# discere-os/zlib.wasm

Hardware: AMD Instinct MI355X
Metric: compress MB/s @ level 6 + CRC32 GB/s, batched 1 MB buffers, 1/2/4/8 GPU (higher is better)
Workload: dtype u8; 1 GPU; C4 per-GPU shard: 32768 x 1048576 B buffers per GPU, deflate level 6, zlib wrapper, inputs+outputs in HBM; level=6, buffer_bytes=1048576, buffers_per_gpu=32768, inflight_mb=4096, parallelism=1 GPU(s), one rank each, buffers sharded by index, no data-path collective, world_size_seen=1

## Files before the change

zlib.wasm_amd/csrc/zgpu_deflate.hip:

```cpp
#include "zgpu_internal.h"
#include <cstdlib>
#include <cstdio>

namespace zgpu {

__constant__ CodeTables c_ct;

constexpr uint32_t kParseFallback = 0xffffffffu;

__device__ inline uint32_t hash3(uint32_t b0, uint32_t b1, uint32_t b2) {
    return ((b0 & 31u) << 10) ^ (b1 << 5) ^ b2;
}
__device__ inline uint32_t hashp(uint32_t b0, uint32_t b1, uint32_t b2, const WinP &w) {
    return ((b0 << (2 * w.shift)) ^ (b1 << w.shift) ^ b2) & w.mask;
}
__device__ inline WinP job_win(const DeflateJob &job) { return win_params(job.wbits, job.hbits); }

__device__ inline uint32_t lds32u(const uint8_t *base, int off) {
    const uint32_t *w = reinterpret_cast<const uint32_t *>(base + (off & ~3));
    return __builtin_amdgcn_alignbyte(w[1], w[0], (uint32_t)(off & 3));
}


template <int kThreads, int kMaxChunksPerThread>
// ... 117 lines not shown
    __syncthreads();
#pragma unroll
    for (int k = 0; k < 4; k++) {
        const int idx = tid * 4 + k;
        wcnt[idx & (kLWaves - 1)][idx >> 4] = (uint16_t)run;
        run += v[k];
    }
    __syncthreads();
#pragma unroll
    for (int j = 0; j < kLPer; j++) {
        const int e = wave * (64 * kLPer) + j * 64 + lane;
        if (e < m) dst[wcnt[wave][(key[j] >> shift) & 0xffu] + rank[j]] = key[j];
    }
    __syncthreads();
}

template <int kC, int kH, bool kSegs, bool kGH>
__device__ __attribute__((always_inline)) inline void links_body(const DeflateJob &job) {
    static_assert(kC <= kLC && (kC & (kC - 1)) == 0 && kC >= 32, "chunk");
    static_assert(!kGH || (!kSegs && kH == 32768), "global head: the default layout, whole buffers");
    __shared__ uint16_t head[kGH ? 1 : kH];
    __shared__ uint32_t ka[kC];
    __shared__ __attribute__((aligned(16))) uint16_t lk[kC];
    uint8_t *const stage = reinterpret_cast<uint8_t *>(lk);
    __shared__ uint16_t wcnt[kLWaves][256];
    __shared__ int wsum[kLWaves];
    const int tid = threadIdx.x;
    const uint32_t bi = kSegs ? job.seg[2 * blockIdx.x] : blockIdx.x;
    const uint32_t g = job.first + bi;
    const int64_t n = (int64_t)job.src_len[g];
    const uint8_t *in = job.src + job.src_off[g];
    uint16_t *out = job.link + job.ws_off[bi];
    const WinP wp = job_win(job);
    const int64_t s0 = kSegs ? (int64_t)job.seg[2 * blockIdx.x + 1] : 0;
    const int64_t s1 = kSegs && s0 + (int64_t)job.seg_len < n ? s0 + (int64_t)job.seg_len : n;
    const int64_t t0 = kSegs && s0 > 32768 ? (s0 - 32768) / kC * kC : 0;

    uint32_t *const ghead = kGH ? reinterpret_cast<uint32_t *>(job.key + job.ws_off[bi]) : nullptr;
    if constexpr (kGH)
        for (int i = tid; i < kH; i += kLThreads) ghead[i] = (uint32_t)-32768;
    else
        for (int i = tid; i < kH; i += kLThreads) head[i] = (uint16_t)((t0 - 32768) & 0xffff);
    const int64_t lk_n = !kSegs && !kGH && job.lk_head ? (int64_t)job.lk_n : 0;
    for (int64_t c0 = t0; c0 < s1; c0 += kC) {
        __syncthreads();
        if (c0 + kC <= lk_n) continue;
        if (kGH) {
        } else if (c0 <= lk_n && job.lk_head) {
            const int hn = (int)wp.mask + 1;
            for (int i = tid; i < kH; i += kLThreads) {
                const int64_t q = i < hn ? (int64_t)job.lk_head[i] : 0;
                head[i] = (uint16_t)(q != 0 && c0 - q < 32768 ? q & 0xffff : (c0 - 32768) & 0xffff);
            }
            __syncthreads();
        } else if ((c0 & 32767) == 0 && c0 > 0) {
            const uint32_t now = (uint32_t)c0;
            for (int i = tid; i < kH; i += kLThreads) {
                const uint32_t age = (now - head[i]) & 0xffffu;
                if (age == 0 || age >= 32768u) head[i] = (uint16_t)((now - 32768u) & 0xffffu);
            }
        }
        stage_bytes<kLThreads, (kC + 16) / 16 / kLThreads + 1>(stage, in, c0, kC + 16, n, tid);
        __syncthreads();
        const int cnt = (int)((n - c0) < kC ? (n - c0) : kC);
        const int m = (int)((n - 2 - c0) < kC ? ((n - 2 - c0) > 0 ? n - 2 - c0 : 0) : kC);
        const int e0 = lk_n > c0 ? (int)(lk_n - c0) : 0;
        const int ms = m > e0 ? m - e0 : 0;
        for (int e = e0 + tid; e < m; e += kLThreads) {
            uint32_t h = hashp(stage[e], stage[e + 1], stage[e + 2], wp);
            if (job.sk.n) {
                const uint32_t p = (uint32_t)c0 + (uint32_t)e;
                for (uint32_t k = 0; k < job.sk.n; k++)
                    if (p >= job.sk.a[k] && p < job.sk.b[k]) h = kSkipHash;
            }
            ka[e - e0] = h << 13 | (uint32_t)e;
        }
        links_radix_pass(ka, ka, ms, 13, wcnt, wsum, tid);
        links_radix_pass(ka, ka, ms, 21, wcnt, wsum, tid);
        for (int i = tid; i < ms; i += kLThreads) {
            const uint32_t key = ka[i];
            const uint32_t h = key >> 13, e = key & (kLC - 1);
            const uint32_t p = (uint32_t)c0 + e;
            uint32_t d;
            if (h == kSkipHash) d = 0;
            else if (i > 0 && (ka[i - 1] >> 13) == h) d = e - (ka[i - 1] & (kLC - 1));
            else if (kGH) d = p - ghead[h];
            else d = (p - head[h]) & 0xffffu;
            lk[e] = (uint16_t)((d != 0 && d <= 32767u && d != p) ? d : 0u);
        }
        __syncthreads();
        for (int i = tid; i < ms; i += kLThreads) {
            const uint32_t key = ka[i];
            if ((key >> 13) != kSkipHash && (i == ms - 1 || (ka[i + 1] >> 13) != (key >> 13))) {
                if (kGH) ghead[key >> 13] = (uint32_t)c0 + (key & (kLC - 1));
                else head[key >> 13] = (uint16_t)(((uint32_t)c0 + (key & (kLC - 1))) & 0xffffu);
            }
        }
        if (kSegs) {
            const int w0 = s0 > c0 ? (int)(s0 - c0) : 0, w1 = (int)(s1 - c0 < cnt ? s1 - c0 : cnt);
            for (int e = tid + w0; e < w1; e += kLThreads) out[c0 + e] = e < m ? lk[e] : (uint16_t)0;
        } else {
            for (int e = tid + e0; e < cnt; e += kLThreads) out[c0 + e] = e < m ? lk[e] : (uint16_t)0;
        }
    }
}

template <int kC, int kH, bool kSegs = false>
__global__ __launch_bounds__(kLThreads) void k_links(DeflateJob job) {
    links_body<kC, kH, kSegs, false>(job);
}

__global__ __launch_bounds__(kLThreads, 8) void k_links_gh(DeflateJob job) {
    links_body<kLC, 32768, false, true>(job);
}

constexpr int kLS1C = 2048;
constexpr int64_t kLS1Max = 16384;
__global__ __launch_bounds__(kLThreads) void k_links_seg1(DeflateJob job) {
    __shared__ uint32_t head[32768];
    __shared__ uint32_t ka[kLS1C];
    __shared__ __attribute__((aligned(16))) uint16_t lk[kLS1C + 16];
    uint8_t *const stage = reinterpret_cast<uint8_t *>(lk);
    __shared__ uint16_t wcnt[kLWaves][256];
    __shared__ int wsum[kLWaves];
    const int tid = threadIdx.x;
    const uint32_t bi = job.seg[2 * blockIdx.x];
    const uint32_t g = job.first + bi;
    const int64_t n = (int64_t)job.src_len[g];
    const uint8_t *in = job.src + job.src_off[g];
    uint16_t *out = job.link + job.ws_off[bi];
    const WinP wp = job_win(job);
    const int64_t s0 = (int64_t)job.seg[2 * blockIdx.x + 1];
    const int64_t s1 = s0 + (int64_t)job.seg_len < n ? s0 + (int64_t)job.seg_len : n;
    auto skipped = [&](int64_t p) {
        for (uint32_t k = 0; k < job.sk.n; k++)
            if ((uint64_t)p >= job.sk.a[k] && (uint64_t)p < job.sk.b[k]) return true;
        return false;
    };
    for (int i = tid; i < 32768; i += kLThreads) head[i] = 0;
    __syncthreads();
    {
        const int64_t w0 = s0 - 32767 > 1 ? s0 - 32767 : 1, w1 = s0 < n - 2 ? s0 : n - 2;
        const int64_t q0 = w0 + 32ll * tid;
        if (q0 < w1) {
            uint32_t wb[9];
            const uintptr_t a = reinterpret_cast<uintptr_t>(in + q0);
            const uint32_t sh = (uint32_t)(a & 3u);
            const uint32_t *qw = reinterpret_cast<const uint32_t *>(a & ~(uintptr_t)3);
            const int64_t lim = n - q0;
            uint32_t d[10];
#pragma unroll
            for (int j = 0; j < 10; j++)
                d[j] = 4ll * j - (int64_t)sh < lim ? qw[j] : 0u;
#pragma unroll
            for (int j = 0; j < 9; j++) wb[j] = sh ? __builtin_amdgcn_alignbyte(d[j + 1], d[j], sh) : d[j];
#pragma unroll
            for (int j = 0; j < 32; j++) {
                const int64_t q = q0 + j;
                if (q >= w1) break;
                const uint32_t b0 = (wb[j >> 2] >> (8 * (j & 3))) & 0xffu;
                const uint32_t b1 = (wb[(j + 1) >> 2] >> (8 * ((j + 1) & 3))) & 0xffu;
                const uint32_t b2 = (wb[(j + 2) >> 2] >> (8 * ((j + 2) & 3))) & 0xffu;
                if (job.sk.n && skipped(q)) continue;
                atomicMax(&head[hashp(b0, b1, b2, wp)], (uint32_t)q + 1u);
            }
        }
    }
    for (int64_t c0 = s0; c0 < s1; c0 += kLS1C) {
        __syncthreads();
        stage_bytes<kLThreads, 1>(stage, in, c0, ((kLS1C + 16) / 16) * 16, n, tid);
        __syncthreads();
        const int cnt = (int)((s1 - c0) < kLS1C ? (s1 - c0) : kLS1C);
        const int m = (int)((n - 2 - c0) < cnt ? ((n - 2 - c0) > 0 ? n - 2 - c0 : 0) : cnt);
        for (int e = tid; e < m; e += kLThreads) {
            uint32_t h = hashp(stage[e], stage[e + 1], stage[e + 2], wp);
            if (job.sk.n && skipped(c0 + e)) h = kSkipHash;
            ka[e] = h << 11 | (uint32_t)e;
        }
        links_radix_pass(ka, ka, m, 11, wcnt, wsum, tid);
        links_radix_pass(ka, ka, m, 19, wcnt, wsum, tid);
        for (int i = tid; i < m; i += kLThreads) {
            const uint32_t key = ka[i];
            const uint32_t h = key >> 11, e = key & (kLS1C - 1);
            const int64_t p = c0 + e;
            int64_t dd;
            if (h == kSkipHash) dd = 0;
            else if (i > 0 && (ka[i - 1] >> 11) == h) dd = e - (ka[i - 1] & (kLS1C - 1));
            else dd = head[h] ? p - ((int64_t)head[h] - 1) : 0;
            lk[e] = (uint16_t)(dd > 0 && dd <= 32767 && dd != p ? dd : 0);
        }
        __syncthreads();
        for (int i = tid; i < m; i += kLThreads) {
            const uint32_t key = ka[i];
            if ((key >> 11) != kSkipHash && (i == m - 1 || (ka[i + 1] >> 11) != (key >> 11)))
                head[key >> 11] = (uint32_t)(c0 + (key & (kLS1C - 1))) + 1u;
        }
        for (int e = tid; e < cnt; e += kLThreads) out[c0 + e] = e < m ? lk[e] : (uint16_t)0;
    }
}

constexpr int kCntStage = 4096;
constexpr int kCntThreads = 1024;

__device__ __attribute__((always_inline)) inline uint32_t walk_key(uint32_t c, uint32_t chain) {
    if (c > chain) c = chain;
    if (c < 128) return c;
    const uint32_t k = 128 + ((c - 128) >> 5);
    return k < 255 ? k : 255;
}

template <bool kSegs = false>
__global__ __launch_bounds__(kCntThreads) void k_count(DeflateJob job) {
    __shared__ uint32_t cnt[16384];
    __shared__ __attribute__((aligned(16))) uint8_t s_in[kCntStage + 16];
    __shared__ __attribute__((aligned(16))) uint8_t s_out[kCntStage + 16];
    const int tid = threadIdx.x;
    const uint32_t bi = kSegs ? job.seg[2 * blockIdx.x] : blockIdx.x;
    const uint32_t g = job.first + bi;
    const int64_t n = (int64_t)job.src_len[g];
    const uint8_t *in = job.src + job.src_off[g];
    uint8_t *key = job.key + job.ws_off[bi];
    const uint32_t chain = job.cfg.chain;
    const int64_t s0 = kSegs ? (int64_t)job.seg[2 * blockIdx.x + 1] : 0;
    const int64_t s1 = kSegs && s0 + (int64_t)job.seg_len < n ? s0 + (int64_t)job.seg_len : n;
    const int64_t c0 = kSegs && s0 > kMaxDist ? (s0 - kMaxDist) / kCntStage * kCntStage : 0;
    for (int i = tid; i < 16384; i += kCntThreads) cnt[i] = 0;
    int64_t tstart = c0;
    if (kSegs && s0 > 0) {
        static_assert(kMaxDist <= 32 * kCntThreads, "one pass");
        __syncthreads();
        const int64_t w0 = s0 - kMaxDist > 1 ? s0 - kMaxDist : 1;
        const int64_t q0 = w0 + 32ll * tid;
        if (q0 < s0) {
            const uintptr_t a = reinterpret_cast<uintptr_t>(in + q0);
            const uint32_t sh = (uint32_t)(a & 3u);
            const uint32_t *qw = reinterpret_cast<const uint32_t *>(a & ~(uintptr_t)3);
            const int64_t lim = n - q0;
            uint32_t d[10], wb[9];
#pragma unroll
            for (int j = 0; j < 10; j++) d[j] = 4ll * j - (int64_t)sh < lim ? qw[j] : 0u;
#pragma unroll
            for (int j = 0; j < 9; j++) wb[j] = sh ? __builtin_amdgcn_alignbyte(d[j + 1], d[j], sh) : d[j];
#pragma unroll
            for (int j = 0; j < 32; j++) {
                const int64_t q = q0 + j;
                if (q >= s0 || q + 3 > n) break;
                const uint32_t h = hash3((wb[j >> 2] >> (8 * (j & 3))) & 0xffu,
                                         (wb[(j + 1) >> 2] >> (8 * ((j + 1) & 3))) & 0xffu,
                                         (wb[(j + 2) >> 2] >> (8 * ((j + 2) & 3))) & 0xffu);
                atomicAdd(&cnt[h >> 1], 1u << ((h & 1u) * 16));
            }
        }
        tstart = s0;
    }
    for (int64_t t0 = tstart; t0 < s1; t0 += kCntStage) {
        __syncthreads();
        stage_bytes<kCntThreads, (kCntStage + 16) / 16 / kCntThreads + 1>(s_in, in, t0, kCntStage + 16, n, tid);
        stage_bytes<kCntThreads, (kCntStage + 16) / 16 / kCntThreads + 1>(s_out, in, t0 - kMaxDist,
                                                                         kCntStage + 16, n, tid);
        __syncthreads();
        const int64_t tend = (t0 + kCntStage < n) ? t0 + kCntStage : n;
        for (int64_t p = t0 + tid; p < tend; p += kCntThreads) {
            const int j = (int)(p - t0);
            const int64_t q = p - kMaxDist;
            if (q >= 1 && q >= c0 && q + 3 <= n) {
                const uint32_t h = hash3(s_out[j], s_out[j + 1], s_out[j + 2]);
                atomicSub(&cnt[h >> 1], 1u << ((h & 1u) * 16));
            }
            uint32_t k = 0;
            if (p >= 1 && p + 3 <= n) {
                const uint32_t h = hash3(s_in[j], s_in[j + 1], s_in[j + 2]);
                const uint32_t old = atomicAdd(&cnt[h >> 1], 1u << ((h & 1u) * 16));
                k = walk_key((old >> ((h & 1u) * 16)) & 0xffffu, chain);
            }
            if (!kSegs || (p >= s0 && p < s1)) key[p] = (uint8_t)k;
        }
    }
}

constexpr int kMW = 32768, kMT = 4096, kMPad = 272;
static_assert(kMT == (int)kMatchTile, "segment starts (host) must be k_match tile boundaries");
constexpr int kME = kMW + kMT + kMPad;
constexpr int kMatchThreads = 1024;

__device__ inline uint32_t get4(const uint32_t *E, int i) {
    return (E[i] >> 16) | (E[i + 2] & 0xffff0000u);
}

__device__ inline uint32_t nil_link(uint32_t l) { return l ? l : 0xffffu; }

static_assert(kMT / 4 == kMatchThreads && kMPad % 4 == 0 && kMPad / 4 <= kMatchThreads && kMW % 4 == 0,
              "tile prefetch: 4 words per thread");
struct TilePre {
    uint32_t b[4];
    uint32_t pb[4];
    uint32_t lk[4];
    uint32_t key[4];
};

__device__ __attribute__((always_inline)) inline uint32_t ldb(const uint8_t *in, int64_t q, int64_t n) {
    return (q >= 0 && q < n) ? (uint32_t)in[q] : 0u;
}

__device__ __attribute__((always_inline)) inline void tile_prefetch(TilePre &P, int64_t ts, int64_t n,
                                                                    const uint8_t *in, const uint16_t *L,
                                                                    const uint8_t *K, int tid) {
    const int64_t q0 = ts + 4 * tid;
    uint32_t x[5];
#pragma unroll
    for (int u = 0; u < 5; u++) x[u] = ldb(in, q0 + u, n);
#pragma unroll
    for (int u = 0; u < 4; u++) P.b[u] = x[u] | x[u + 1] << 8;
    if (tid < kMPad / 4) {
        const int64_t q1 = ts + kMT + 4 * tid;
#pragma unroll
        for (int u = 0; u < 5; u++) x[u] = ldb(in, q1 + u, n);
#pragma unroll
        for (int u = 0; u < 4; u++) P.pb[u] = x[u] | x[u + 1] << 8;
    }
    if (q0 + 4 <= n) {
        const uint2 v = *reinterpret_cast<const uint2 *>(L + q0);
        P.lk[0] = v.x & 0xffffu; P.lk[1] = v.x >> 16; P.lk[2] = v.y & 0xffffu; P.lk[3] = v.y >> 16;
    } else {
#pragma unroll
        for (int u = 0; u < 4; u++) P.lk[u] = q0 + u < n ? (uint32_t)L[q0 + u] : 0u;
    }
    if (K) {
#pragma unroll
        for (int u = 0; u < 4; u++) {
            const int64_t q = ts + tid + u * kMatchThreads;
            P.key[u] = q < n ? (uint32_t)K[q] : 0u;
        }
    }
}

__device__ __attribute__((always_inline)) inline uint32_t slide_idx(uint32_t w) {
    typedef unsigned short us2 __attribute__((ext_vector_type(2)));
    const us2 v = __builtin_bit_cast(us2, w);
    const us2 d = {(unsigned short)kMT, (unsigned short)0};
    return __builtin_bit_cast(uint32_t, __builtin_elementwise_sub_sat(v, d));
}
template <bool kIdx = false>
__device__ __attribute__((always_inline)) inline void tile_store(uint32_t *E, const TilePre &P, int64_t ts,
                                                                 int tid) {
    if (ts == 0) {
        for (int i = tid; i < kMW; i += kMatchThreads) E[i] = 0;
    } else {
        uint4 *dE = reinterpret_cast<uint4 *>(E);
        for (int c = tid; c < kMW / 4; c += kMatchThreads) {
            uint4 v = dE[c + kMT / 4];
            if (kIdx) v = make_uint4(slide_idx(v.x), slide_idx(v.y), slide_idx(v.z), slide_idx(v.w));
            dE[c] = v;
        }
        __syncthreads();
    }
    const int w0 = kMW + 4 * tid;
    uint4 v;
    if (kIdx) {
        v.x = P.b[0] << 16 | (P.lk[0] ? ((uint32_t)(w0 + 0) - P.lk[0]) & 0xffffu : 0u);
        v.y = P.b[1] << 16 | (P.lk[1] ? ((uint32_t)(w0 + 1) - P.lk[1]) & 0xffffu : 0u);
        v.z = P.b[2] << 16 | (P.lk[2] ? ((uint32_t)(w0 + 2) - P.lk[2]) & 0xffffu : 0u);
        v.w = P.b[3] << 16 | (P.lk[3] ? ((uint32_t)(w0 + 3) - P.lk[3]) & 0xffffu : 0u);
    } else {
        v.x = P.b[0] << 16 | nil_link(P.lk[0]);
        v.y = P.b[1] << 16 | nil_link(P.lk[1]);
        v.z = P.b[2] << 16 | nil_link(P.lk[2]);
        v.w = P.b[3] << 16 | nil_link(P.lk[3]);
    }
    *reinterpret_cast<uint4 *>(E + w0) = v;
    if (tid < kMPad / 4)
        *reinterpret_cast<uint4 *>(E + kMW + kMT + 4 * tid) =
            make_uint4(P.pb[0] << 16, P.pb[1] << 16, P.pb[2] << 16, P.pb[3] << 16);
}

struct Scan16 { uint32_t s0, s1, s2, s3; };


constexpr int kD0 = 2;
constexpr int kDQ = 6;
constexpr int kDU = 3;
__device__ inline uint32_t ufl(uint32_t v) { return (uint32_t)__builtin_amdgcn_readfirstlane((int)v); }

__device__ __attribute__((always_inline)) inline uint32_t get4p(const uint32_t *E, int i) {
    return __builtin_amdgcn_perm(E[i + 2], E[i], 0x07060302u);
}

__device__ __attribute__((always_inline)) inline uint32_t ffbl(uint32_t x) {
    uint32_t r;
    asm("v_ffbl_b32 %0, %1" : "=v"(r) : "v"(x));
    return r;
}

__device__ __attribute__((always_inline)) inline int diff16(uint32_t x0, uint32_t x1, uint32_t x2, uint32_t x3) {
    const uint32_t b = min(min(ffbl(x0), ffbl(x1) | 32u), min(ffbl(x2) | 64u, ffbl(x3) | 96u));
    return (int)(min(b, 128u) >> 3);
}

__device__ __attribute__((always_inline)) inline int lcp16(const uint32_t *E, int m, int s, const Scan16 &S,
                                                           int maxcmp) {
    int k = diff16(get4p(E, m) ^ S.s0, get4p(E, m + 4) ^ S.s1, get4p(E, m + 8) ^ S.s2, get4p(E, m + 12) ^ S.s3);
    if (k >= 16) {
        while (k < maxcmp) {
            const int r = diff16(get4p(E, m + k) ^ get4p(E, s + k), get4p(E, m + k + 4) ^ get4p(E, s + k + 4),
                                 get4p(E, m + k + 8) ^ get4p(E, s + k + 8), get4p(E, m + k + 12) ^ get4p(E, s + k + 12));
            k += r;
            if (r < 16) break;
        }
    }
    return k < maxcmp ? k : maxcmp;
}
__device__ __attribute__((always_inline)) inline void lcp16x2(const uint32_t *E, int m1, int m0, int s,
                                                              const Scan16 &S, int maxcmp, int &l1, int &l0) {
    const uint32_t a0 = get4p(E, m1) ^ S.s0, a1 = get4p(E, m1 + 4) ^ S.s1, a2 = get4p(E, m1 + 8) ^ S.s2,
                   a3 = get4p(E, m1 + 12) ^ S.s3;
    const uint32_t b0 = get4p(E, m0) ^ S.s0, b1 = get4p(E, m0 + 4) ^ S.s1, b2 = get4p(E, m0 + 8) ^ S.s2,
                   b3 = get4p(E, m0 + 12) ^ S.s3;
    int k1 = diff16(a0, a1, a2, a3), k0 = diff16(b0, b1, b2, b3);
    auto more = [&](int m, int k) {
        while (k < maxcmp) {
            const int r = diff16(get4p(E, m + k) ^ get4p(E, s + k), get4p(E, m + k + 4) ^ get4p(E, s + k + 4),
                                 get4p(E, m + k + 8) ^ get4p(E, s + k + 8), get4p(E, m + k + 12) ^ get4p(E, s + k + 12));
            k += r;
            if (r < 16) break;
        }
        return k;
    };
    if (k1 >= 16) k1 = more(m1, k1);
    if (k0 >= 16) k0 = more(m0, k0);
    l1 = k1 < maxcmp ? k1 : maxcmp;
    l0 = k0 < maxcmp ? k0 : maxcmp;
}
__device__ inline uint32_t match_rec(int best, int s4, int bpos4) {
    return best >= kMinMatch ? (((uint32_t)best << 16) | (uint32_t)((s4 - bpos4) >> 2)) : 0u;
}


#ifdef ZGPU_MATCH_STATS
__device__ unsigned long long g_mstat[8];
#define MSTAT(i, v) atomicAdd(&g_mstat[i], (unsigned long long)(v))
#define MSTATW(i, v) do { if ((int)__lane_id() == __builtin_ctzll(__ballot(1))) atomicAdd(&g_mstat[i], (unsigned long long)(v)); } while (0)
extern "C" int zgpu_match_stats_read(unsigned long long *out, int reset) {
    if (hipMemcpyFromSymbol(out, HIP_SYMBOL(g_mstat), sizeof(g_mstat)) != hipSuccess) return -1;
    if (reset) {
        unsigned long long z[8] = {0, 0, 0, 0, 0, 0, 0, 0};
        if (hipMemcpyToSymbol(HIP_SYMBOL(g_mstat), z, sizeof(z)) != hipSuccess) return -1;
    }
    return 0;
}
#endif

struct DWQ {
    int m4, limit4, be4, occ;
    int q[kDQ];
    uint32_t em, eb, scan01, scanE;
};
__device__ __attribute__((always_inline)) inline void dwq_steps(DWQ &w, const char *Eb, uint32_t &count,
                                                                uint32_t end) {
    auto step = [&]() {
        const int m4n = (int)((w.em << 2) & 0x3fffcu);
        const uint32_t emn = *reinterpret_cast<const uint32_t *>(Eb + m4n);
        const uint32_t ebn = *reinterpret_cast<const uint32_t *>(Eb + m4n + w.be4);
        const bool pass = (w.m4 > w.limit4) & ((w.em >> 16) == w.scan01) & ((w.eb >> 16) == w.scanE);
#pragma unroll
        for (int j = kDQ - 1; j > 0; j--) w.q[j] = pass ? w.q[j - 1] : w.q[j];
        w.q[0] = pass ? w.m4 : w.q[0];
        w.occ += pass ? 1 : 0;
        w.m4 = m4n;
        w.em = emn;
        w.eb = ebn;
    };
    for (;;) {
        if (end - count >= (uint32_t)kDU) {
#pragma unroll
            for (int u = 0; u < kDU; u++) step();
            count += kDU;
        } else {
            step();
            count += 1;
        }
        const uint64_t walkers = __ballot(w.m4 > w.limit4), full = __ballot(w.occ >= kDQ - (kDU - 1));
        if (count >= end || walkers == 0 || full != 0) break;
    }
}

constexpr uint32_t kQDiff = 1u << 31;
struct MOutRQ {
    uint32_t *rf, *rq;
    int64_t p;
    mutable uint32_t q = 0;
    mutable bool hq = false;
    __device__ __attribute__((always_inline)) inline void full(uint32_t r, bool) const {
        const bool d = hq && q != r;
        if (d) rq[p] = q;
        rf[p] = d ? r | kQDiff : r;
    }
    __device__ __attribute__((always_inline)) inline void quart(uint32_t r) const {
        q = r;
        hq = true;
    }
    __device__ __attribute__((always_inline)) inline void steps(uint32_t) const {}
};
template <typename Out>
__device__ __attribute__((always_inline)) inline void dwq_walk(const uint32_t *E, int64_t p, int64_t B, int64_t n,
                                                               const LevelCfg &cfg, const Out &out,
                                                               int want_q, int64_t max_dist) {
    const int s = (int)(p - B);
    const uint32_t e0 = E[s];
    const uint32_t d0 = (e0 & 0xffffu) ? (uint32_t)s - (e0 & 0xffffu) : 0xffffu;
    if (d0 > (uint32_t)max_dist) {
        if (want_q) out.quart(0u);
        out.full(0u, true);
        return;
    }
    const int64_t labs = p > max_dist ? p - max_dist : 0;
    const int limit4 = (int)(labs - B) * 4;
    const int64_t rem = n - p;
    const int nice = rem < cfg.nice ? (int)rem : cfg.nice;
    const int maxcmp = rem < kMaxMatch ? (int)rem : kMaxMatch;
    const uint32_t chain = (uint32_t)cfg.chain;
    const uint32_t qc = want_q ? chain >> 2 : chain;
    const int s4 = s * 4;
    const Scan16 S{get4(E, s), get4(E, s + 4), get4(E, s + 8), get4(E, s + 12)};
    int best = kMinMatch - 1, bpos4 = 0;
    int m4 = (int)(e0 & 0xffffu) * 4;
    uint32_t count = 0;
    bool walking = true;
    bool need_q = want_q != 0;
#pragma unroll
    for (int k = 0; k < kD0; k++) {
        if (walking) {
            const int m = m4 >> 2;
            const uint32_t em = E[m];
            const int len = lcp16(E, m, s, S, maxcmp);
            if (len > best) { best = len; bpos4 = m4; }
            count++;
            const int m4n = (int)((em & 0xffffu) << 2);
            if (best >= nice || m4n <= limit4 || count >= chain) walking = false;
            if (need_q && count == qc && walking) {
                out.quart(match_rec(best, s4, bpos4));
                need_q = false;
            }
            m4 = m4n;
        }
    }
    if (!walking) {
        const uint32_t r = match_rec(best, s4, bpos4);
        if (need_q) out.quart(r);
        out.steps(count);
        out.full(r, best >= nice || m4 <= limit4);
        return;
    }
    const char *Eb = reinterpret_cast<const char *>(E);
#ifdef ZGPU_MATCH_STATS
    MSTATW(4, 1);
    MSTAT(6, 1);
#endif
    DWQ w;
    w.m4 = m4;
    w.limit4 = limit4;
    w.be4 = (best - 1) * 4;
    w.occ = 0;
#pragma unroll
    for (int j = 0; j < kDQ; j++) w.q[j] = 0;
    w.scan01 = e0 >> 16;
    w.scanE = E[s + best - 1] >> 16;
    w.em = *reinterpret_cast<const uint32_t *>(Eb + m4);
    w.eb = *reinterpret_cast<const uint32_t *>(Eb + m4 + w.be4);
    count = ufl(count);
    for (;;) {
        const uint32_t end = count < qc ? qc : chain;
        const int best0 = best;
        dwq_steps(w, Eb, count, end);
        walking = w.m4 > limit4 && count < chain;
#ifdef ZGPU_MATCH_STATS
        MSTATW(0, 1);
        MSTAT(2, (uint64_t)w.occ);
        MSTAT(3, 1);
#endif
        static_assert(kDQ % 2 == 0, "entries are taken in pairs");
#pragma unroll
        for (int j = kDQ - 1; j >= 1; j -= 2) {
            const bool c1 = j < w.occ, c0 = j - 1 < w.occ;
            if (__ballot(c0) != 0) {
                int l1, l0;
                lcp16x2(E, c1 ? w.q[j] >> 2 : 0, c0 ? w.q[j - 1] >> 2 : 0, s, S, maxcmp, l1, l0);
#ifdef ZGPU_MATCH_STATS
                MSTATW(1, 1);
                MSTAT(5, (c1 && l1 >= 16 ? 1 : 0) + (c0 && l0 >= 16 ? 1 : 0));
#endif
                if (c1 && l1 > best) {
                    best = l1;
                    bpos4 = w.q[j];
                    if (l1 >= nice) { walking = false; w.occ = 0; }
                }
                if (c0 && j - 1 < w.occ && l0 > best) {
                    best = l0;
                    bpos4 = w.q[j - 1];
                    if (l0 >= nice) { walking = false; w.occ = 0; }
                }
            }
        }
        w.occ = 0;
        const bool fin = !walking;
        if (need_q && (count >= qc || fin)) {
            out.quart(match_rec(best, s4, bpos4));
            need_q = false;
        }
        if (fin) break;
        if (best != best0) {
            w.be4 = (best - 1) * 4;
            w.scanE = E[s + best - 1] >> 16;
            w.eb = *reinterpret_cast<const uint32_t *>(Eb + w.m4 + w.be4);
        }
    }
    out.steps(count);
    out.full(match_rec(best, s4, bpos4), best >= nice || w.m4 <= limit4);
}


struct FlushEv {
    const uint64_t *pos;
    const uint32_t *type;
    const uint64_t *aux;
    uint32_t n, i;
    __device__ inline bool at(int64_t p) const {
        return i < n && kind() != 0 && kind() != kEvPause && kind() != kEvPrime && (int64_t)ufl64(pos[i]) == p;
    }
    __device__ inline bool prime() const { return i < n && kind() == kEvPrime; }
    __device__ inline uint32_t prime_arg() const { return (uint32_t)ufl64(aux[i]); }
    __device__ inline bool stop_at(int64_t e, int64_t lim) const { return i < n && kind() == 0 && e == lim; }
    __device__ inline bool pause_at(int64_t x) const {
        return i < n && kind() == kEvPause && (int64_t)ufl64(aux[i]) == x;
    }
    __device__ inline uint32_t kind() const { return (uint32_t)__builtin_amdgcn_readfirstlane((int)type[i]); }
    __device__ inline int64_t limit(int64_t end) const { return i < n ? (int64_t)ufl64(pos[i]) : end; }
    __device__ static inline uint64_t ufl64(uint64_t v) {
        const uint32_t lo = (uint32_t)__builtin_amdgcn_readfirstlane((int)(uint32_t)v);
        const uint32_t hi = (uint32_t)__builtin_amdgcn_readfirstlane((int)(uint32_t)(v >> 32));
        return ((uint64_t)hi << 32) | lo;
    }
};
__device__ inline FlushEv flush_ev(const DeflateJob &job) { return FlushEv{job.fl_pos, job.fl_type, job.fl_aux, job.nfl, 0}; }

__device__ inline int64_t flush_limit(const DeflateJob &job, int64_t p, int64_t n) {
    uint32_t lo = 0, hi = job.nmlim;
    while (lo < hi) {
        const uint32_t mid = (lo + hi) >> 1;
        if ((int64_t)job.mlim[mid] > p) hi = mid;
        else lo = mid + 1;
    }
    return lo < job.nmlim ? (int64_t)job.mlim[lo] : n;
}

__device__ inline uint32_t cfg_count(const DeflateJob &job, int64_t p) {
    uint32_t k = 0;
    while (k < job.ncfg && (int64_t)job.cfg_pos[k] <= p) k++;
    return k;
}
__device__ inline LevelCfg cfg_row(const DeflateJob &job, uint32_t k) { return k ? job.cfg_tab[k - 1] : job.cfg; }

template <bool kEv = false, bool kSegs = false>
__global__ __launch_bounds__(kMatchThreads) void k_match(DeflateJob job, int want_q) {
    constexpr int kSortBuckets = 64;
    __shared__ __attribute__((aligned(16))) uint32_t E[kME];
    __shared__ int next_i;
    __shared__ uint16_t s_perm[kMT];
    __shared__ int s_hist[kSortBuckets], s_base[kSortBuckets];
    const int tid = threadIdx.x;
    const uint32_t bi = kSegs ? job.seg[2 * blockIdx.x] : blockIdx.x;
    const uint32_t g = job.first + bi;
    const int64_t n = (int64_t)job.src_len[g];
    const int64_t s0 = kSegs ? (int64_t)job.seg[2 * blockIdx.x + 1] : 0;
    const int64_t s1 = kSegs && s0 + (int64_t)job.seg_len < n ? s0 + (int64_t)job.seg_len : n;
    const int64_t t0 = kSegs && s0 > kMW ? s0 - kMW : 0;
    const uint8_t *in = job.src + job.src_off[g];
    const uint16_t *L = job.link + job.ws_off[bi];
    uint32_t *rf = job.rfull + job.ws_off[bi];
    uint32_t *rq = job.rquart + job.ws_off[bi];
    const uint8_t *K = job.key + job.ws_off[bi];
    const LevelCfg cfg = job.cfg;
    const int64_t max_dist = job_win(job).max_dist;

    const bool one_shot = kSegs && s0 > 0;
    const int64_t tstart = one_shot ? s0 : t0;
    if (one_shot) {
        const int64_t wb = s0 - kMW;
        constexpr int kQuads = (kME + 4 * kMatchThreads - 1) / (4 * kMatchThreads);
        constexpr int kBatch = 5;
        static_assert(kQuads <= 2 * kBatch, "two batches of quad loads");
#pragma unroll
        for (int b0 = 0; b0 < kQuads; b0 += kBatch) {
            uint32_t x[kBatch][5], lk[kBatch][4];
#pragma unroll
            for (int u = 0; u < kBatch; u++) {
                const int w = 4 * (tid + (b0 + u) * kMatchThreads);
                const int64_t q = wb + w;
#pragma unroll
                for (int v = 0; v < 5; v++) x[u][v] = ldb(in, q + v, n);
                if (w < kMW + kMT && q >= 0 && q + 4 <= n) {
                    const uint2 t = *reinterpret_cast<const uint2 *>(L + q);
                    lk[u][0] = t.x & 0xffffu; lk[u][1] = t.x >> 16; lk[u][2] = t.y & 0xffffu; lk[u][3] = t.y >> 16;
                } else {
#pragma unroll
                    for (int v = 0; v < 4; v++)
                        lk[u][v] = w < kMW + kMT && q + v >= 0 && q + v < n ? (uint32_t)L[q + v] : 0u;
                }
            }
#pragma unroll
            for (int u = 0; u < kBatch; u++) {
                const int w = 4 * (tid + (b0 + u) * kMatchThreads);
                if (b0 + u >= kQuads || w >= kME) continue;
#pragma unroll
                for (int v = 0; v < 4; v++) {
                    const uint32_t l = lk[u][v];
                    const uint32_t wi = (uint32_t)(w + v);
                    E[w + v] = (x[u][v] | x[u][v + 1] << 8) << 16 | (l && wi >= l ? (wi - l) & 0xffffu : 0u);
                }
            }
        }
    }
    TilePre P;
    tile_prefetch(P, tstart, n, in, L, K, tid);
    for (int64_t ts = tstart; ts < s1; ts += kMT) {
        const int64_t B = ts - kMW;
        const int tile_n = kSegs && ts < s0 ? 0 : (int)((n - ts) < kMT ? (n - ts) : kMT);
        if (!(one_shot && ts == tstart)) tile_store<true>(E, P, ts, tid);
        if (tid == 0) next_i = 0;
        if (tid < kSortBuckets) s_hist[tid] = 0;
        __syncthreads();
        int bk[4], rk[4];
#pragma unroll
        for (int u = 0; u < 4; u++) {
            const int i = tid + u * kMatchThreads;
            bk[u] = kSortBuckets - 1 - (i < tile_n ? (int)(P.key[u] >> 2) : 0);
        }
#pragma unroll
        for (int u = 0; u < 4; u++)
            rk[u] = tid + u * kMatchThreads < tile_n ? atomicAdd(&s_hist[bk[u]], 1) : 0;
        __syncthreads();
        if (tid < 64) {
            const int v = s_hist[tid];
            int incl = v;
#pragma unroll
            for (int o = 1; o < 64; o <<= 1) {
                const int t = __shfl_up(incl, o, 64);
                if (tid >= o) incl += t;
            }
            s_base[tid] = incl - v;
        }
        __syncthreads();
#pragma unroll
        for (int u = 0; u < 4; u++)
            if (tid + u * kMatchThreads < tile_n)
                s_perm[s_base[bk[u]] + rk[u]] = (uint16_t)(tid + u * kMatchThreads);
        __syncthreads();
        if (ts + kMT < s1) tile_prefetch(P, ts + kMT, n, in, L, K, tid);
        const uint32_t k0 = kEv && tile_n ? cfg_count(job, ts) : 0;
        const uint32_t k1 = kEv && tile_n ? cfg_count(job, ts + tile_n - 1) : 0;
        for (uint32_t k = k0; k <= k1; k++) {
            const LevelCfg c = kEv ? cfg_row(job, k) : cfg;
            const int64_t lo = k ? (int64_t)job.cfg_pos[k - 1] : -1;
            const int64_t hi = kEv && k < job.ncfg ? (int64_t)job.cfg_pos[k] : INT64_MAX;
            if (k > k0) {
                __syncthreads();
                if (tid == 0) next_i = 0;
                __syncthreads();
            }
            for (;;) {
                const int i = atomicAdd(&next_i, 1);
                if (i >= tile_n) break;
                const int64_t p = ts + (int)s_perm[i];
                if (kEv && (p < lo || p >= hi)) continue;
                const int64_t nl = kEv ? flush_limit(job, p, n) : n;
                dwq_walk(E, p, B, nl, c, MOutRQ{rf, rq, p}, want_q, max_dist);
            }
        }
        __syncthreads();
    }
}

__device__ inline uint32_t vg(uint32_t x) {
    return (uint32_t)__builtin_amdgcn_update_dpp(0, (int)x, 0xE4, 0xF, 0xF, false);
}

template <typename P>
struct ParseOutT {
    uint32_t *sym;
    BlockRec *blk;
    uint32_t nsym, blk_nsym, blk_sym_start, nblk;
    P block_start, S, E;
    P wsize, max_dist;
    uint32_t sym_limit;
    bool lead;
    bool vaddr = false;
    uint64_t *srec = nullptr;

    __device__ inline void rec(P strstart, bool res) {
        if (lead && srec) {
            srec[4ull * nblk + 2] = ((uint64_t)S << 32) | (uint64_t)strstart;
            srec[4ull * nblk + 3] = (uint64_t)E | (res ? 1ull << 63 : 0ull);
        }
    }

    __device__ inline void win(const WinP &w) { wsize = w.wsize; max_dist = w.max_dist; sym_limit = w.sym_limit; }
    __device__ inline bool tally(uint32_t v) {
        if (vaddr) sym[vg(nsym)] = v;
        else if (lead) sym[nsym] = v;
        nsym++;
        return ++blk_nsym == sym_limit;
    }
    __device__ inline void flush(P strstart, bool last) {
        BlockRec r;
        r.sym_start = blk_sym_start;
        r.nsym = blk_nsym;
        r.in_start = (uint64_t)block_start;
        r.in_end = (uint64_t)strstart;
        r.flags = (last ? 1u : 0u) | (block_start >= S ? 2u : 0u);
        r.pad = 0;
        if (lead) blk[nblk] = r;
        rec(strstart, true);
        nblk++;
        block_start = strstart;
        blk_sym_start = nsym;
        blk_nsym = 0;
    }
    __device__ inline void marker(P strstart, uint32_t kind, uint32_t arg = 0) {
        BlockRec r;
        r.sym_start = blk_sym_start;
        r.nsym = 0;
        r.in_start = r.in_end = (uint64_t)strstart;
        r.flags = kBlkMarker | (kind << 4);
        r.pad = arg;
        if (lead) blk[nblk] = r;
        rec(strstart, kind != kMarkPrime);
        nblk++;
    }
    __device__ inline void fill(P p, P n) {
        if (p - S >= wsize + max_dist) S += wsize;
        if (E < n) { P e = S + 2 * wsize; E = e < n ? e : n; }
    }
};
using ParseOut = ParseOutT<int64_t>;


constexpr int kPT = 4096;


struct ParseU {
    uint32_t *sym;
    BlockRec *blk;
    uint32_t nsym, blk_nsym, blk_sym_start, nblk;
    uint32_t block_start, S, E;
    uint32_t wsize, max_dist, sym_limit;
    uint64_t *srec;
    __device__ inline void rec(uint32_t strstart, bool res, int lane) {
        if (lane == 0 && srec) {
            srec[4ull * nblk + 2] = ((uint64_t)S << 32) | strstart;
            srec[4ull * nblk + 3] = (uint64_t)E | (res ? 1ull << 63 : 0ull);
        }
    }
    __device__ inline void flush(uint32_t strstart, bool last, int lane, bool res = true) {
        rec(strstart, res, lane);
        if (lane == 0) {
            BlockRec r;
            r.sym_start = blk_sym_start;
            r.nsym = blk_nsym;
            r.in_start = block_start;
            r.in_end = strstart;
            r.flags = (last ? 1u : 0u) | (block_start >= S ? 2u : 0u);
            r.pad = 0;
            blk[nblk] = r;
        }
        nblk++;
        block_start = strstart;
        blk_sym_start = nsym;
        blk_nsym = 0;
    }
    __device__ inline bool tally1(uint32_t v, int lane) {
        if (lane == 0) sym[nsym] = v;
        nsym++;
        return ++blk_nsym == sym_limit;
    }
    __device__ inline void marker(uint32_t strstart, uint32_t kind, int lane, uint32_t arg = 0) {
        if (lane == 0) {
            BlockRec r;
            r.sym_start = blk_sym_start;
            r.nsym = 0;
            r.in_start = r.in_end = strstart;
            r.flags = kBlkMarker | (kind << 4);
            r.pad = arg;
            blk[nblk] = r;
        }
        rec(strstart, kind != kMarkPrime, lane);
        nblk++;
    }
    __device__ inline void fill(uint32_t p, uint32_t n) {
        if (p - S >= wsize + max_dist) S += wsize;
        if (E < n) { uint32_t e = S + 2 * wsize; E = e < n ? e : n; }
    }
};

__device__ uint32_t walk_best0(const uint8_t *in, const uint16_t *lk, uint32_t p, uint32_t n, uint32_t lookahead,
                               uint32_t S, uint32_t max_dist, const LevelCfg &cfg, uint32_t *ms, bool *searched,
                               int lane) {
    const uint32_t d0 = lk[p];
    *searched = d0 != 0 && d0 <= max_dist;
    if (!*searched) return kMinMatch - 1;
    uint32_t chain = cfg.good == 0 ? cfg.chain >> 2 : cfg.chain;
    const uint32_t nice = lookahead < cfg.nice ? lookahead : cfg.nice;
    const uint32_t limit = p - S > max_dist ? p - max_dist : S;
    const uint32_t maxcmp = n - p < (uint32_t)kMaxMatch ? n - p : (uint32_t)kMaxMatch;
    int best = 0;
    uint32_t cur = p - d0, start = 0;
    for (;;) {
        const bool pass = in[cur + best] == in[p + best] && in[cur + best - 1] == in[p + best - 1] &&
                          in[cur] == in[p] && in[cur + 1] == in[p + 1];
        if (pass) {
            uint32_t len = maxcmp;
            for (uint32_t k0 = 0; k0 < maxcmp; k0 += 64) {
                const uint32_t k = k0 + (uint32_t)lane;
                const uint64_t m = __ballot(k < maxcmp && in[cur + k] != in[p + k]);
                if (m) { len = k0 + (uint32_t)__builtin_ctzll(m); break; }
            }
            if ((int)len > best) {
                start = cur;
                best = (int)len;
                if (len >= nice) break;
            }
        }
        const uint32_t d = lk[cur];
        if (d == 0 || d >= cur - limit || --chain == 0) break;
        cur -= d;
    }
    *ms = start;
    return (uint32_t)best <= lookahead ? (uint32_t)best : lookahead;
}

template <int kT>
__global__ __launch_bounds__(64) void k_parse_slow(DeflateJob job, int only_flagged) {
    __shared__ __attribute__((aligned(16))) uint32_t s_rf[kT];
    __shared__ __attribute__((aligned(16))) uint8_t s_in[kT + 16];
    const int lane = threadIdx.x;
    const uint32_t bi = blockIdx.x;
    const uint32_t g = job.first + bi;
    const uint32_t n = (uint32_t)job.src_len[g];
    const uint8_t *in = job.src + job.src_off[g];
    const uint32_t *rf = job.rfull + job.ws_off[bi];
    const uint32_t *rq = job.rquart + job.ws_off[bi];
    const LevelCfg cfg = job.cfg;
    bool use_q = cfg.good < cfg.lazy;
    const bool filtered = job.strategy == 1;
    uint32_t lazy = cfg.lazy, good = cfg.good;
    uint32_t ci = 0;
    if (only_flagged && job.nblocks[bi] != kParseFallback) return;

    ParseU po;
    po.sym = job.sym + job.ws_off[bi];
    po.blk = job.blocks + job.blk_off[bi];
    po.nsym = po.blk_nsym = po.blk_sym_start = po.nblk = 0;
    {
        const WinP wp = job_win(job);
        po.wsize = (uint32_t)wp.wsize; po.max_dist = (uint32_t)wp.max_dist; po.sym_limit = wp.sym_limit;
    }
    uint32_t p = job.start, match_start = 0, match_length = job.srec ? (uint32_t)job.zm0 : kMinMatch - 1;
    uint32_t zprev = job.srec ? (uint32_t)job.zp0 : kMinMatch - 1;
    const uint16_t *lk = job.link + job.ws_off[bi];
    po.block_start = p; po.S = 0; po.E = job.e0 > p ? job.e0 : p;
    po.srec = job.srec;
    bool avail = false, done = false;
    FlushEv fe = flush_ev(job);
    while (fe.prime()) {
        if (lane == 0 && job.ev_blk) job.ev_blk[fe.i] = po.nblk;
        po.marker(p, kMarkPrime, lane, fe.prime_arg());
        fe.i++;
    }
    uint32_t lim = (uint32_t)fe.limit(n);

    uint32_t t0 = p & ~15u;
    while (!done) {
        stage_words<64, kT / 4 / 64>(s_rf, rf, t0, kT, n, lane);

        stage_bytes<64, (kT + 16) / 16 / 64 + 1>(s_in, in, (int64_t)t0 - 16, kT + 16, n, lane);
        __syncthreads();
        const bool tile_to_end = (uint64_t)t0 + kT >= n;
        for (;;) {
            if (!tile_to_end && p + 64 > t0 + kT) break;
            if (p > po.E) { done = true; break; }
            if (po.E - p < (uint32_t)kMinLookahead) {
                po.fill(p, lim);
                while (fe.stop_at(po.E, lim) && po.E - p < (uint32_t)kMinLookahead) {
                    if (lane == 0 && job.ev_blk) job.ev_blk[fe.i] = po.nblk;
                    fe.i++;
                    while (fe.prime()) {
                        if (lane == 0 && job.ev_blk) job.ev_blk[fe.i] = po.nblk;
                        po.marker(p, kMarkPrime, lane, fe.prime_arg());
                        fe.i++;
                    }
                    if (fe.i == fe.n && job.open_end) { done = true; break; }
                    lim = (uint32_t)fe.limit(n);
                    po.fill(p, lim);
                }
                if (done) break;
                if (po.E == p) {
                    if (fe.at(p)) {
                        if (avail) po.tally1(ufl(s_in[p - 1 - t0 + 16]), lane);
                        avail = false;
                        match_length = kMinMatch - 1;
                        if (po.blk_nsym) po.flush(p, false, lane);
                        if (lane == 0 && job.ev_blk) job.ev_blk[fe.i] = po.nblk;
                        po.marker(p, fe.kind(), lane);
                        if (lane == 0 && job.flush_out) job.flush_out[2] = po.S;
                        fe.i++;
                        lim = (uint32_t)fe.limit(n);
                        continue;
                    }
                    done = true;
                    break;
                }
            }
            const uint32_t lookahead = po.E - p;
            if (match_length < kMinMatch && match_length != 0 && p + 64 + kMinLookahead <= po.E) {
                const uint32_t r = s_rf[p - t0 + lane] & ~kQDiff;
                const uint32_t rl = r >> 16;
                const bool hit = rl >= kMinMatch &&
                                 !(rl <= 5u && (filtered || (rl == kMinMatch && (r & 0xffffu) > (uint32_t)kTooFar)));
                const uint64_t mask = __ballot(hit);
                const uint32_t k = mask ? (uint32_t)__builtin_ctzll(mask) : 64u;
                if (k > 0) {
                    uint32_t a = avail ? p - 1 : p;
                    const uint32_t b = p + k - 1;
                    while (a < b) {
                        const uint32_t room = po.sym_limit - po.blk_nsym;
                        const uint32_t take = (b - a) < room ? (b - a) : room;
                        if ((uint32_t)lane < take) po.sym[po.nsym + lane] = s_in[a + lane - t0 + 16];
                        po.nsym += take;
                        po.blk_nsym += take;
                        a += take;
                        if (po.blk_nsym == po.sym_limit) {
                            po.flush(a, false, lane);
                            if (fe.pause_at(a)) {
                                if (lane == 0 && job.ev_blk) job.ev_blk[fe.i] = po.nblk;
                                fe.i++;
                                while (fe.prime()) {
                                    if (lane == 0 && job.ev_blk) job.ev_blk[fe.i] = po.nblk;
                                    po.marker(a, kMarkPrime, lane, fe.prime_arg());
                                    fe.i++;
                                }
                                lim = (uint32_t)fe.limit(n);
                            }
                        }
                    }
                    avail = true;
                    p += k;
                    zprev = kMinMatch - 1;
                    continue;
                }
            }
            while (ci < job.ncfg && p >= (uint32_t)job.cfg_pos[ci]) {
                lazy = job.cfg_tab[ci].lazy;
                good = job.cfg_tab[ci].good;
                use_q = good < lazy;
                ci++;
            }
            const uint32_t prev_length = match_length, prev_match = match_start;
            zprev = prev_length;
            match_length = kMinMatch - 1;
            if (lookahead >= kMinMatch && prev_length < lazy) {
                if (prev_length == 0) {
                    uint32_t ms = 0;
                    bool searched = false;
                    const uint32_t ml = walk_best0(in, lk, p, n, lookahead, po.S, po.max_dist, LevelCfg{good, lazy,
                                                   ci ? job.cfg_tab[ci - 1].nice : cfg.nice,
                                                   ci ? job.cfg_tab[ci - 1].chain : cfg.chain}, &ms, &searched, lane);
                    if (searched) {
                        match_length = ml;
                        match_start = ms;
                        if (match_length <= 5u && (filtered || (match_length == kMinMatch && p - match_start > (uint32_t)kTooFar)))
                            match_length = kMinMatch - 1;
                    }
                } else {
                    const uint32_t w = ufl(s_rf[p - t0]);
// ... 4102 lines not shown
```

Baseline: 10620 MB/s.

## Cut barriers and atomics in match tile setup with wave-aggregated bucket sort

```diff
diff --git a/zlib.wasm_amd/csrc/zgpu_deflate.hip b/zlib.wasm_amd/csrc/zgpu_deflate.hip
--- a/zlib.wasm_amd/csrc/zgpu_deflate.hip
+++ b/zlib.wasm_amd/csrc/zgpu_deflate.hip
@@ -443,22 +443,31 @@
     return (q >= 0 && q < n) ? (uint32_t)in[q] : 0u;
 }
 
+__device__ __attribute__((always_inline)) inline void ldw4(uint32_t *b, const uint8_t *in, int64_t q, int64_t n,
+                                                           bool wide) {
+    if (wide && q + 8 <= n) {
+        const uint32_t *p = reinterpret_cast<const uint32_t *>(in + q);
+        const uint32_t d0 = p[0], d1 = p[1];
+        b[0] = d0 & 0xffffu;
+        b[1] = (d0 >> 8) & 0xffffu;
+        b[2] = d0 >> 16;
+        b[3] = (d0 >> 24) | (d1 & 0xffu) << 8;
+    } else {
+        uint32_t x[5];
+#pragma unroll
+        for (int u = 0; u < 5; u++) x[u] = ldb(in, q + u, n);
+#pragma unroll
+        for (int u = 0; u < 4; u++) b[u] = x[u] | x[u + 1] << 8;
+    }
+}
+
 __device__ __attribute__((always_inline)) inline void tile_prefetch(TilePre &P, int64_t ts, int64_t n,
                                                                     const uint8_t *in, const uint16_t *L,
                                                                     const uint8_t *K, int tid) {
     const int64_t q0 = ts + 4 * tid;
-    uint32_t x[5];
-#pragma unroll
-    for (int u = 0; u < 5; u++) x[u] = ldb(in, q0 + u, n);
-#pragma unroll
-    for (int u = 0; u < 4; u++) P.b[u] = x[u] | x[u + 1] << 8;
-    if (tid < kMPad / 4) {
-        const int64_t q1 = ts + kMT + 4 * tid;
-#pragma unroll
-        for (int u = 0; u < 5; u++) x[u] = ldb(in, q1 + u, n);
-#pragma unroll
-        for (int u = 0; u < 4; u++) P.pb[u] = x[u] | x[u + 1] << 8;
-    }
+    const bool wide = (reinterpret_cast<uintptr_t>(in) & 7u) == 0;
+    ldw4(P.b, in, q0, n, wide);
+    if (tid < kMPad / 4) ldw4(P.pb, in, ts + kMT + 4 * tid, n, wide);
     if (q0 + 4 <= n) {
         const uint2 v = *reinterpret_cast<const uint2 *>(L + q0);
         P.lk[0] = v.x & 0xffffu; P.lk[1] = v.x >> 16; P.lk[2] = v.y & 0xffffu; P.lk[3] = v.y >> 16;
@@ -467,10 +476,12 @@
         for (int u = 0; u < 4; u++) P.lk[u] = q0 + u < n ? (uint32_t)L[q0 + u] : 0u;
     }
     if (K) {
+        const int tn = (int)(n - ts < kMT ? n - ts : kMT);
+        const uint8_t *Kt = K + ts;
 #pragma unroll
         for (int u = 0; u < 4; u++) {
-            const int64_t q = ts + tid + u * kMatchThreads;
-            P.key[u] = q < n ? (uint32_t)K[q] : 0u;
+            const int i = tid + u * kMatchThreads;
+            P.key[u] = i < tn ? (uint32_t)Kt[i] : 0u;
         }
     }
 }
@@ -488,12 +499,16 @@
         for (int i = tid; i < kMW; i += kMatchThreads) E[i] = 0;
     } else {
         uint4 *dE = reinterpret_cast<uint4 *>(E);
-        for (int c = tid; c < kMW / 4; c += kMatchThreads) {
-            uint4 v = dE[c + kMT / 4];
-            if (kIdx) v = make_uint4(slide_idx(v.x), slide_idx(v.y), slide_idx(v.z), slide_idx(v.w));
-            dE[c] = v;
-        }
-        __syncthreads();
+        constexpr int kCh = kMW / 4 / kMatchThreads;
+        static_assert(kCh * kMatchThreads * 4 == kMW && kMT / 4 == kMatchThreads, "a thread's chunks are its own");
+        uint4 v[kCh];
+#pragma unroll
+        for (int j = 0; j < kCh; j++) v[j] = dE[tid + (j + 1) * (kMT / 4)];
+#pragma unroll
+        for (int j = 0; j < kCh; j++) {
+            if (kIdx) v[j] = make_uint4(slide_idx(v[j].x), slide_idx(v[j].y), slide_idx(v[j].z), slide_idx(v[j].w));
+            dE[tid + j * kMatchThreads] = v[j];
+        }
     }
     const int w0 = kMW + 4 * tid;
     uint4 v;
@@ -576,14 +591,14 @@
 }
 
 
-#ifdef ZGPU_MATCH_STATS
-__device__ unsigned long long g_mstat[8];
+#if defined(ZGPU_MATCH_STATS) || defined(ZGPU_MATCH_CLOCK)
+__device__ unsigned long long g_mstat[12];
 #define MSTAT(i, v) atomicAdd(&g_mstat[i], (unsigned long long)(v))
 #define MSTATW(i, v) do { if ((int)__lane_id() == __builtin_ctzll(__ballot(1))) atomicAdd(&g_mstat[i], (unsigned long long)(v)); } while (0)
 extern "C" int zgpu_match_stats_read(unsigned long long *out, int reset) {
     if (hipMemcpyFromSymbol(out, HIP_SYMBOL(g_mstat), sizeof(g_mstat)) != hipSuccess) return -1;
     if (reset) {
-        unsigned long long z[8] = {0, 0, 0, 0, 0, 0, 0, 0};
+        unsigned long long z[12] = {0, 0, 0, 0, 0, 0, 0, 0, 0, 0, 0, 0};
         if (hipMemcpyToSymbol(HIP_SYMBOL(g_mstat), z, sizeof(z)) != hipSuccess) return -1;
     }
     return 0;
@@ -594,6 +609,9 @@
     int m4, limit4, be4, occ;
     int q[kDQ];
     uint32_t em, eb, scan01, scanE;
+#ifdef ZGPU_MATCH_STATS
+    uint32_t ls;
+#endif
 };
 __device__ __attribute__((always_inline)) inline void dwq_steps(DWQ &w, const char *Eb, uint32_t &count,
                                                                 uint32_t end) {
@@ -602,6 +620,9 @@
         const uint32_t emn = *reinterpret_cast<const uint32_t *>(Eb + m4n);
         const uint32_t ebn = *reinterpret_cast<const uint32_t *>(Eb + m4n + w.be4);
         const bool pass = (w.m4 > w.limit4) & ((w.em >> 16) == w.scan01) & ((w.eb >> 16) == w.scanE);
+#ifdef ZGPU_MATCH_STATS
+        w.ls += w.m4 > w.limit4 ? 1 : 0;
+#endif
 #pragma unroll
         for (int j = kDQ - 1; j > 0; j--) w.q[j] = pass ? w.q[j - 1] : w.q[j];
         w.q[0] = pass ? w.m4 : w.q[0];
@@ -670,6 +691,10 @@
 #pragma unroll
     for (int k = 0; k < kD0; k++) {
         if (walking) {
+#ifdef ZGPU_MATCH_STATS
+            MSTATW(10, 1);
+            MSTAT(11, 1);
+#endif
             const int m = m4 >> 2;
             const uint32_t em = E[m];
             const int len = lcp16(E, m, s, S, maxcmp);
@@ -701,6 +726,9 @@
     w.limit4 = limit4;
     w.be4 = (best - 1) * 4;
     w.occ = 0;
+#ifdef ZGPU_MATCH_STATS
+    w.ls = 0;
+#endif
 #pragma unroll
     for (int j = 0; j < kDQ; j++) w.q[j] = 0;
     w.scan01 = e0 >> 16;
@@ -711,10 +739,14 @@
     for (;;) {
         const uint32_t end = count < qc ? qc : chain;
         const int best0 = best;
+#ifdef ZGPU_MATCH_STATS
+        const uint32_t count0 = count;
+#endif
         dwq_steps(w, Eb, count, end);
         walking = w.m4 > limit4 && count < chain;
 #ifdef ZGPU_MATCH_STATS
         MSTATW(0, 1);
+        MSTATW(10, count - count0);
         MSTAT(2, (uint64_t)w.occ);
         MSTAT(3, 1);
 #endif
@@ -754,6 +786,9 @@
             w.eb = *reinterpret_cast<const uint32_t *>(Eb + w.m4 + w.be4);
         }
     }
+#ifdef ZGPU_MATCH_STATS
+    MSTAT(11, w.ls);
+#endif
     out.steps(count);
     out.full(match_rec(best, s4, bpos4), best >= nice || w.m4 <= limit4);
 }
@@ -806,7 +841,7 @@
     __shared__ __attribute__((aligned(16))) uint32_t E[kME];
     __shared__ int next_i;
     __shared__ uint16_t s_perm[kMT];
-    __shared__ int s_hist[kSortBuckets], s_base[kSortBuckets];
+    __shared__ int s_hist[kSortBuckets];
     const int tid = threadIdx.x;
     const uint32_t bi = kSegs ? job.seg[2 * blockIdx.x] : blockIdx.x;
     const uint32_t g = job.first + bi;
@@ -862,39 +897,65 @@
     }
     TilePre P;
     tile_prefetch(P, tstart, n, in, L, K, tid);
+    if (tid == 0) next_i = 0;
+    if (tid < kSortBuckets) s_hist[tid] = 0;
+    __syncthreads();
+#ifdef ZGPU_MATCH_CLOCK
+    unsigned long long ck_tile = 0, ck_walk = 0;
+#endif
     for (int64_t ts = tstart; ts < s1; ts += kMT) {
+#ifdef ZGPU_MATCH_CLOCK
+        const unsigned long long ck0 = wall_clock64();
+#endif
         const int64_t B = ts - kMW;
         const int tile_n = kSegs && ts < s0 ? 0 : (int)((n - ts) < kMT ? (n - ts) : kMT);
         if (!(one_shot && ts == tstart)) tile_store<true>(E, P, ts, tid);
-        if (tid == 0) next_i = 0;
-        if (tid < kSortBuckets) s_hist[tid] = 0;
-        __syncthreads();
         int bk[4], rk[4];
 #pragma unroll
         for (int u = 0; u < 4; u++) {
             const int i = tid + u * kMatchThreads;
             bk[u] = kSortBuckets - 1 - (i < tile_n ? (int)(P.key[u] >> 2) : 0);
         }
-#pragma unroll
-        for (int u = 0; u < 4; u++)
-            rk[u] = tid + u * kMatchThreads < tile_n ? atomicAdd(&s_hist[bk[u]], 1) : 0;
+        {
+            const int lane = tid & 63;
+            const uint64_t below = (1ull << lane) - 1ull;
+#pragma unroll
+            for (int u = 0; u < 4; u++) {
+                const bool act = tid + u * kMatchThreads < tile_n;
+                uint64_t peers = __ballot(act);
+#pragma unroll
+                for (int b = 0; b < 6; b++) {
+                    const uint64_t bb = __ballot((bk[u] >> b) & 1);
+                    peers &= ((bk[u] >> b) & 1) ? bb : ~bb;
+                }
+                int base = 0;
+                if (act && (peers & below) == 0) base = atomicAdd(&s_hist[bk[u]], __popcll(peers));
+                base = __shfl(base, act ? __builtin_ctzll(peers) : lane, 64);
+                rk[u] = act ? base + __popcll(peers & below) : 0;
+            }
+        }
         __syncthreads();
-        if (tid < 64) {
-            const int v = s_hist[tid];
+        {
+            const int lane = tid & 63;
+            const int v = s_hist[lane];
             int incl = v;
 #pragma unroll
             for (int o = 1; o < 64; o <<= 1) {
                 const int t = __shfl_up(incl, o, 64);
-                if (tid >= o) incl += t;
-            }
-            s_base[tid] = incl - v;
+                if (lane >= o) incl += t;
+            }
+            const int excl = incl - v;
+#pragma unroll
+            for (int u = 0; u < 4; u++) {
+                const int base = __shfl(excl, bk[u], 64);
+                if (tid + u * kMatchThreads < tile_n) s_perm[base + rk[u]] = (uint16_t)(tid + u * kMatchThreads);
+            }
         }
         __syncthreads();
-#pragma unroll
-        for (int u = 0; u < 4; u++)
-            if (tid + u * kMatchThreads < tile_n)
-                s_perm[s_base[bk[u]] + rk[u]] = (uint16_t)(tid + u * kMatchThreads);
-        __syncthreads();
+        if (tid < kSortBuckets) s_hist[tid] = 0;
+#ifdef ZGPU_MATCH_CLOCK
+        const unsigned long long ck1 = wall_clock64();
+#endif
         if (ts + kMT < s1) tile_prefetch(P, ts + kMT, n, in, L, K, tid);
         const uint32_t k0 = kEv && tile_n ? cfg_count(job, ts) : 0;
         const uint32_t k1 = kEv && tile_n ? cfg_count(job, ts + tile_n - 1) : 0;
@@ -917,7 +978,18 @@
             }
         }
         __syncthreads();
-    }
+        if (tid == 0) next_i = 0;
+#ifdef ZGPU_MATCH_CLOCK
+        ck_tile += ck1 - ck0;
+        ck_walk += wall_clock64() - ck1;
+#endif
+    }
+#ifdef ZGPU_MATCH_CLOCK
+    if (tid == 0) {
+        MSTAT(8, ck_tile);
+        MSTAT(9, ck_walk);
+    }
+#endif
 }
 
 __device__ inline uint32_t vg(uint32_t x) {
```

Result: no change. 10660 MB/s, median of 6 (+0.4%).
